# naver-ai/egtr

Hardware: AMD Instinct MI355X
Metric: images/sec end-to-end SGG, 600x1000 input, N=200 queries (higher is better)
Workload: dtype f32; 1 GPU; VG inference: ResNet-50, N=200, 6 enc/6 dec, 150 classes, 50 predicates, 600x1000, bs=1/GPU fp32 (BASELINE configs[1]); hip_graph=True, gemm_tuning=True, miopen_find=True, parallelism=replicas x1 (independent images, no collective)

## Files before the change

### egtr_amd/_lib.py

```python
import ctypes
import os

import torch

_HERE = os.path.dirname(os.path.abspath(__file__))
LIB_PATH = os.environ.get("EGTR_HIP_LIBRARY") or os.path.join(_HERE, "libegtr_hip.so")

_P = ctypes.c_void_p
_I = ctypes.c_int
ABI_VERSION = 5

SIGNATURES = {
    "egtr_abi_version": [],
    "egtr_status_string": [_I],
    "egtr_last_hip_error": [],
    "egtr_msda_forward_f32": [_P, _P, _P, _P, _P, _P, _I, _I, _I, _I, _I, _I, _I, _P],
    "egtr_msda_forward_fused_vbias_f32": [_P, _P, _P, _P, _P, _P, _P, _I, _I, _I, _I, _I, _I, _I, _P, _P, _I, _I, _P, _P,
                                          _P],
    "egtr_msda_forward_fused_box_f32": [_P, _P, _P, _P, _P, _P, _P, _I, _I, _I, _I, _I, _I, _I, _P, _P, _I, _I, _P, _P,
                                        _P],
    "egtr_msda_backward_f32": [_P, _P, _P, _P, _P, _P, _P, _I, _I, _I, _I, _I, _I, _I, _P, _P, _P],
    "egtr_msda_backward_out_f32": [_P, _P, _P, _P, _P, _P, _P, _I, _I, _I, _I, _I, _I, _I, _P, _P, _P],
    "egtr_msda_forward_f64": [_P, _P, _P, _P, _P, _P, _I, _I, _I, _I, _I, _I, _I, _P],
    "egtr_msda_backward_f64": [_P, _P, _P, _P, _P, _P, _P, _I, _I, _I, _I, _I, _I, _I, _P, _P, _P],
# ... 50 lines not shown
                           _I, _P, _P, _P, _P],
    "egtr_oi_match_f32": [_P, _P, _P, _I, _I, _P, _P, _I, _I, _P, _P, ctypes.c_longlong, _P, _P, _P, ctypes.c_longlong,
                          _P, _I, _P, _P, _P],
    "egtr_oi_ap_f64": [_P, _P, _P, _P, ctypes.c_longlong, _I, _P, _P],
    "egtr_coco_match_f32": [_P, _P, _P, _P, _I, _I, _I, _P, _P, _P, _P, _P, ctypes.c_longlong, _P, _P, _I, _P, _P, _P,
                            _P, _P],
    "egtr_coco_accumulate_f64": [_P, _P, _P, _P, _P, ctypes.c_longlong, _I, _P, _P, _P, _P],
    "egtr_hungarian_match_f32": [_P, _P, _P, _P, _P, _P, _P, _I, _I, _I, _I, ctypes.c_float, ctypes.c_float,
                                 ctypes.c_float, _I, ctypes.c_float, ctypes.c_float, _P, _P, _P, _P, _P, _P, _P],
    "egtr_hungarian_match_scratch_doubles": [_I, _I, ctypes.c_longlong],
    "egtr_add_layernorm_backward_f32": [_P, _P, _P, _P, _P, _P, _P, _P, _I, _I, ctypes.c_float],
    "egtr_add_layernorm_backward_workspace_floats": [_I],
    "egtr_msda_geometry_forward_f32": [_P, _P, ctypes.c_longlong, _P, ctypes.c_longlong, _P, _I, _P, _P, _P, ctypes.c_longlong, _I, _I, _I],
    "egtr_msda_geometry_backward_f32": [_P, _P, _P, _P, _P, ctypes.c_longlong, _P, _I, _P, _P, ctypes.c_longlong, _P, ctypes.c_longlong, _P, ctypes.c_longlong, _I, _I, _I],
    "egtr_linear_backward_f32": [_P, _P, _P, _P, _P, ctypes.c_float, _P, _P, _P, _I, _I, _I],
    "egtr_linear_backward_acc_f32": [_P, _P, _P, _P, _P, ctypes.c_float, _P, _P, _P, _I, _I, _I, _P, _P],
    "egtr_weighted_column_sum_f32": [_P, _P, _P, _P, _P, _I, _I],
    "egtr_column_sum_f32": [_P, _P, _P, _P, _P, _P, _I, _I],
    "egtr_column_sum_workspace_floats": [_I, _I],
    "egtr_any_nonfinite_f32": [_P, _P, ctypes.c_longlong, _P],
    "egtr_clamp_if_flag_f32": [_P, _P, _P, ctypes.c_longlong, _P, ctypes.c_float, _I],
    "egtr_detection_loss_f32": [_P, _P, _P, _P, _P, _P, _P, _P, _P, _I, _I, _I, ctypes.c_float, ctypes.c_float, _P, _P,
                                _P, _P],
    "egtr_relation_loss_f32": [_P, _P, _P, _P, _P, _P, _P, _P, _I, _I, _I, ctypes.c_float, _I, _I, _P, _P, _P, _P],
    "egtr_relation_loss_workspace_bytes": [_I, _I],
    "egtr_relation_loss_bits_f32": [_P, _P, _P, _P, _P, _P, _P, _P, _I, _I, _I, ctypes.c_float, _I, _I, _P, _P, _P, _P],
    "egtr_pack_relations_u64": [_P, _P, _P, _I, _I, _I, _I, _P],
    "egtr_rel_head_forward_bf16w": [_P] * 16 + [_I] * 6 + [_P] * 3,
    "egtr_ffn_layernorm_bf16": [_P] * 7 + [ctypes.c_float, _P, _I, _P, _P, _I, _I, _I],
    "egtr_ffn_pack_weights_bf16": [_P, _P, _P, _I, _I, _P],
    "egtr_ffn_packed_weights_bytes": [_I],
    "egtr_linear_bf16": [_P, _P, _I, _P, _P, _P, _I, _I, _I, _I, _I, ctypes.c_float],
    "egtr_rel_head_forward_bf16p": [_P] * 16 + [_I] * 6 + [_P] * 3,
    "egtr_rel_head_pack_tables_bf16": [_P, _P, _I, _I, _I, _P],
    "egtr_linear_split_bf16_f32": [_P, _P, _I, _P, _P, _P, _I, _I, _I, _I, _I],
    "egtr_linear_split_bf16_wgrad_f32": [_P, _P, _I, _P, _I, _P, _P, _I, _I, _I],
    "egtr_linear_split_bf16_wgrad_workspace_floats": [_I, _I, _I],
    "egtr_gemm_split_tile_weights_f32": [_P, _P, _I, _I, _I, _I, _P],
    "egtr_gemm_split_tile_weights_pair_f32": [_P, _P, _I, _I, _I, _P],
    "egtr_gemm_split_tile_weights_multi_f32": [_P, _I, _P, _P, _P, _P, _P, _P, _P, _P],
    "egtr_linear_split_bf16_grouped_pos_f32": [_P, _I, _P, _P, _P, _P, _P, _P, _P, _P, _I, _I, _P, _P],
    "egtr_linear_split_bf16_ex_f32": [_P, _I, _P, _P, _P, _P, _P, _P, _P, _P, _I, _I, _P, _P, _P, _P, _P, _P, _P, _P, _P],
    "egtr_linear_split_bf16_wgrad_ex_f32": [_P, _P, _I, _P, _I, _P, _P, _I, _I, _I, _P, _I, _P],
    "egtr_dropout_add_layernorm_f32": [_P, _P, _P, _P, ctypes.c_float, _P, _P, _P, _I, _I, ctypes.c_float, _P],
    "egtr_dropout_add_layernorm_backward_workspace_floats": [_I],
    "egtr_dropout_add_layernorm_backward_f32": [_P, _P, _P, _P, ctypes.c_float, _P, _P, _P, _P, ctypes.c_float, _P, _P, _P,
                                                _P, _I, _I, ctypes.c_float],
    "egtr_pad_batch_f32": [_P, _P, _P, _I, _I, _I, _I, _P, _P],
    "egtr_preprocess_f32": [_P, _P, _I, _P, _P, _I, _I, _I, _I, _P, _P, _P],
    "egtr_preprocess_bf16": [_P, _P, _I, _P, _P, _I, _I, _I, _I, _P, _P, _P],
    "egtr_preprocess_augment_f32": [_P, _P, _P, _I, _P, _P, _I, _I, _I, _I, _I, _I, _I, _I, _P, _P, _P],
    "egtr_preprocess_augment_bf16": [_P, _P, _P, _I, _P, _P, _I, _I, _I, _I, _I, _I, _I, _I, _P, _P, _P],
    "egtr_conv1x1_tail_x6_f32": [_P, _P, _I, _P, _I, _P, _P, _P, _I, _I, _P, _I, _I, _I, _I, _I, _I],
    "egtr_stem_conv7x7_pool_bf16": [_P, _P, _P, _P, _P, _I, _I, _I],
    "egtr_stem_conv7x7_pool_x6_f32": [_P, _P, _P, _P, _P, _I, _I, _I],
    "egtr_conv1x1_strided_x6_f32": [_P, _P, _P, _P, _I, _I, _I, _I, _I, _I],
    "egtr_conv3x3_phase_channels": [_I, _I, _I, _I],
    "egtr_conv3x3_x6_f32": [_P, _P, _P, _P, _I, _I, _I, _I, _I, _I, _I],
    "egtr_conv3x3_x6_shift_f32": [_P, _P, _P, _P, _P, _I, _I, _I, _I, _I, _I, _I],
    "egtr_conv1x1_tail_pack_weights_bf16": [_P, _P, _I, _I, _I, _P],
    "egtr_conv1x1_tail_bf16": [_P, _P, _I, _P, _I, _P, _P, _P, _I, _I, _P, _I, _I, _I, _I],
    "egtr_ffn_x6_f32": [_P, _P, _I, _P, _P, _P, _P, _P, _P, ctypes.c_float, _P, _I, _P, _P, _I, _I, _I],
    "egtr_encoder_tail_x6_f32": [_P, _P, _I, _P, _I, _P, _P, _P, _P, ctypes.c_float, _P, _P, _P, _P, _P, _P, ctypes.c_float,
                                 _P, _I, _P, _P, _I, _I, _I],
    "egtr_proj_ln_x6_f32": [_P, _P, _I, _P, _P, _P, _I, _P, _P, ctypes.c_float, _P, _I, _P, _P, _I, _I],
    "egtr_proj_multi_x6_f32": [_P, _P, _I, _P, _P, _P, _I, _I, _I],
    "egtr_xs_bytes": [_I, _I],
    "egtr_xs_split_f32": [_P, _P, _I, _P, _I, _I, _I, _P, _P, _I],
    "egtr_rel_head_forward_bf16x6_f32": [_P] * 16 + [_I] * 6 + [_P] * 3 + [_I],
    "egtr_rel_head_forward_bf16x6_save_f32": [_P] * 16 + [_I] * 6 + [_P] * 5,
    "egtr_rel_head_streams_f32": [_P] * 4 + [_I] * 2 + [_P] * 3,
    "egtr_rel_head_forward_save_f32": [_P] * 16 + [_I] * 6 + [_P] * 5,
    "egtr_rel_head_backward_pairs_f32": [_P] * 6 + [_I] * 4 + [_P] * 5,
    "egtr_decoder_layer_f32": [_P, _P],
    "egtr_decoder_layer_workspace": [_I, _I, _P, _P, _P],
}
_RESTYPES = {"egtr_status_string": ctypes.c_char_p, "egtr_last_hip_error": ctypes.c_char_p,
             "egtr_ffn_packed_weights_bytes": ctypes.c_longlong,
             "egtr_input_proj_groupnorm_tokens_workspace_floats": ctypes.c_longlong,
             "egtr_msda_backward_bf16_workspace_floats": ctypes.c_longlong,
             "egtr_hungarian_match_scratch_doubles": ctypes.c_longlong,
             "egtr_relation_loss_workspace_bytes": ctypes.c_longlong,
             "egtr_column_sum_workspace_floats": ctypes.c_longlong,
             "egtr_add_layernorm_backward_workspace_floats": ctypes.c_longlong,
             "egtr_linear_split_bf16_wgrad_workspace_floats": ctypes.c_longlong,
             "egtr_dropout_add_layernorm_backward_workspace_floats": ctypes.c_longlong,
             "egtr_xs_bytes": ctypes.c_longlong, "egtr_sgg_eval_width": ctypes.c_longlong,
             "egtr_oi_eval_width": ctypes.c_longlong, "egtr_matched_topk_workspace_bytes": ctypes.c_longlong, "egtr_oi_select_workspace_bytes": ctypes.c_longlong}

_lib = None


class EgtrHipError(RuntimeError):
    pass


def lib():
    global _lib
    if _lib is None:
        if not os.path.exists(LIB_PATH):
            raise EgtrHipError(
                f"{LIB_PATH} not found: the HIP extension has not been built "
                "(run `make -C egtr_amd/csrc` or __graft_entry__.build()). There is no CPU fallback.")
        handle = ctypes.CDLL(LIB_PATH)
        handle.egtr_abi_version.restype = ctypes.c_int
        got = handle.egtr_abi_version()
# ... 60 lines not shown
```

### egtr_amd/backbone.py

```python
import os

import torch
import torch.nn.functional as F
from torch import nn


TRAIN_FUSED_EPILOGUE = True
NHWC_BF16 = os.environ.get("EGTR_BACKBONE_NHWC", "1") != "0"
NHWC_F32 = os.environ.get("EGTR_BACKBONE_NHWC", "1") != "0"
CONV3_FUSED = True
CONV3_FUSED_BF16 = True
CONV1_X6 = True
CONV1_X6_SHAPES = ((64, 64),)
CONV1_SHIFT_ON_LOAD = True
CONV1_PLAIN_SHAPES = ((256, 64), (256, 128), (512, 128), (1024, 256))
CONV1_SPLIT_SHAPES = ()
SHORTCUT_X6 = True
FROZEN_PREFIX_NHWC = True
STEM_FUSED_BF16 = True
STEM_FUSED = True
CONV2_X6 = True
CONV2_X6_MAX_WIDTH = 512


def _fold(conv, bn):
    scale = bn.weight.float() * (bn.running_var.float() + 1e-5).rsqrt()
    shift = bn.bias.float() - bn.running_mean.float() * scale
    return ((conv.weight.float() * scale.reshape(-1, 1, 1, 1)).to(conv.weight.dtype).contiguous(),
            shift.contiguous())


def conv1x1_as_gemm(x, weight):
    b, c, h, w_ = x.shape
    return torch.matmul(weight.reshape(weight.shape[0], c), x.reshape(b, c, h * w_)).view(b, -1, h, w_)


class DeformableDetrFrozenBatchNorm2d(nn.Module):

    def __init__(self, n):
        super().__init__()
        self.register_buffer("weight", torch.ones(n))
        self.register_buffer("bias", torch.zeros(n))
        self.register_buffer("running_mean", torch.zeros(n))
        self.register_buffer("running_var", torch.ones(n))

    def _load_from_state_dict(self, state_dict, prefix, local_metadata, strict, missing_keys, unexpected_keys,
                              error_msgs):
        state_dict.pop(prefix + "num_batches_tracked", None)
        super()._load_from_state_dict(state_dict, prefix, local_metadata, strict, missing_keys, unexpected_keys,
                                      error_msgs)

    def forward(self, x):
        scale = self.weight * (self.running_var + 1e-5).rsqrt()
        shift = self.bias - self.running_mean * scale
        return x * scale.reshape(1, -1, 1, 1) + shift.reshape(1, -1, 1, 1)


class ScaleWeightsFunction(torch.autograd.Function):

    @staticmethod
    def forward(ctx, scales, *weights):
        from . import ops
        ctx.scales = scales
        return tuple(ops.scale_rows_multi([w.detach() for w in weights], scales))

    @staticmethod
    def backward(ctx, *grads):
        from . import ops
        present = [i for i, g in enumerate(grads) if g is not None]
        out = [None] * len(grads)
# ... 86 lines not shown
        w2, b2 = p[1]
        w3, b3 = p[2]
        out = {"w1": w1.reshape(w1.shape[0], -1).contiguous(), "b1": b1.to(w1.dtype).contiguous(),
               "w2": w2.contiguous(memory_format=torch.channels_last), "b2": b2,
               "w3": w3.reshape(w3.shape[0], -1).contiguous(), "b3": b3, "wd": None}
        if self.downsample is not None:
            wd = p[3][0]
            out["wd"] = (wd.reshape(wd.shape[0], -1).contiguous() if tuple(self.downsample[0].stride) == (1, 1)
                         else wd.contiguous(memory_format=torch.channels_last))
            out["b3"] = p[4][1]
        return out

    def forward_folded_nhwc(self, x, q):
        from . import ops
        B, C, H, W_ = x.shape
        x2 = x.permute(0, 2, 3, 1).reshape(-1, C)
        N1 = q["w1"].shape[0]
        st2 = tuple(self.conv2.stride)
        conv2_x6 = (CONV2_X6 and ops.GEMM_SPLIT_BF16 and st2 in ((1, 1), (2, 2)) and q["w2"].shape[0] <= CONV2_X6_MAX_WIDTH)
        shift1 = None
        if (CONV1_X6 and ops.GEMM_SPLIT_BF16 and (C, N1) in CONV1_X6_SHAPES and ops.conv1x1_tail_supported(x2, N1)):
            if "w1xs" not in q:
                q["w1xs"] = ops.xs_split(q["w1"], weights=True)
                q["b1f"] = q["b1"].float().contiguous()
            y = ops.conv1x1_tail(x2, None, q["w1xs"], q["b1f"], None, N1, relu_in=False, relu_out=True)
        elif (CONV1_SHIFT_ON_LOAD and conv2_x6 and (C, N1) in CONV1_PLAIN_SHAPES and x.is_cuda and x.dtype == torch.float32
              and q["b1"].dtype == torch.float32 and N1 == q["w2"].shape[1]):
            if (C, N1) in CONV1_SPLIT_SHAPES and ops.gemm_split_supported(x2, N1, C):
                if "w1gs" not in q:
                    q["w1gs"] = ops.gemm_split_weights(q["w1"])
                y = ops.linear_split_bf16(x2, q["w1gs"], None, N1)
            else:
                y = torch.mm(x2, q["w1"].t())
            shift1 = q["b1"]
        else:
            y = torch._addmm_activation(q["b1"], x2, q["w1"].t(), use_gelu=False)
        y = y.view(B, H, W_, -1).permute(0, 3, 1, 2)
        conv2_x6 = conv2_x6 and ops.conv3x3_supported(y, q["w2"].shape[0], st2[0])
        if shift1 is not None and not conv2_x6:
            ops.bias_act_rows_(y.permute(0, 2, 3, 1).reshape(-1, N1), shift1)
            shift1 = None
        if conv2_x6:
            if "w2xs" not in q:
                q["w2xs"] = ops.conv3x3_weights(q["w2"], st2[0])
            y = ops.conv3x3(y, q["w2xs"], q["w2"].shape[0], st2[0], in_shift=shift1)
        else:
            y = F.conv2d(y, q["w2"], None, stride=self.conv2.stride, padding=1)
        if not y.is_contiguous(memory_format=torch.channels_last):
            ops.note_fallback("backbone_nhwc", "a channels-last convolution returned an NCHW tensor: "
                              "PYTORCH_MIOPEN_SUGGEST_NHWC=1 was not set before the process's first convolution")
        Ho, Wo = y.shape[-2:]
        y2 = y.permute(0, 2, 3, 1).reshape(-1, y.shape[1])
        N3 = q["w3"].shape[0]
        if self.downsample is None:
            idt = x2
        elif q["wd"].dim() == 2:
            idt = torch.mm(x2, q["wd"].t())
        elif (SHORTCUT_X6 and ops.GEMM_SPLIT_BF16 and tuple(self.downsample[0].stride) == (2, 2)
              and ops.conv1x1_strided_supported(x, N3, 2)):
            if "wdxs" not in q:
                q["wdxs"] = ops.xs_split(q["wd"].reshape(N3, C).contiguous(), weights=True)
            idt = ops.conv1x1_strided(x, q["wdxs"], N3, 2)
        else:
            idt = F.conv2d(x, q["wd"], None, stride=self.downsample[0].stride).permute(0, 2, 3, 1).reshape(-1, N3)
        if (CONV3_FUSED and ops.GEMM_SPLIT_BF16 and ops.conv1x1_tail_supported(y2, N3) and idt.dtype == torch.float32
                and idt.stride(1) == 1 and idt.stride(0) % 4 == 0 and idt.data_ptr() % 16 == 0):
            if "w3xs" not in q:
                q["w3xs"] = ops.xs_split(q["w3"], weights=True)
            z = ops.conv1x1_tail(y2, q["b2"], q["w3xs"], q["b3"], idt, N3)
            return z.view(B, Ho, Wo, -1).permute(0, 3, 1, 2)
        if (CONV3_FUSED_BF16 and ops.conv1x1_tail_bf16_supported(y2, N3) and idt.dtype == torch.bfloat16 and idt.stride(1) == 1
                and idt.stride(0) % 8 == 0 and idt.data_ptr() % 16 == 0):
            if "w3pk" not in q:
                q["w3pk"] = ops.conv_tail_pack_bf16(q["w3"])
            z = ops.conv1x1_tail_bf16(y2, q["b2"], q["w3pk"], q["b3"], idt, N3)
            return z.view(B, Ho, Wo, -1).permute(0, 3, 1, 2)
        ops.bias_act_rows_(y2, q["b2"])
        z = torch.mm(y2, q["w3"].t())
        ops.bias_act_rows_(z, q["b3"], idt)
        return z.view(B, Ho, Wo, -1).permute(0, 3, 1, 2)

    def forward_folded(self, x, p):
        from . import ops
        s = self.conv2.stride
        idt = x
        shift3 = p[2][1]
        if self.downsample is not None:
            if tuple(self.downsample[0].stride) == (1, 1):
                idt = conv1x1_as_gemm(x, p[3][0])
            else:
                idt = F.conv2d(x, p[3][0], None, stride=self.downsample[0].stride)
            shift3 = p[4][1]
        y = ops.bias_act_(conv1x1_as_gemm(x, p[0][0]), p[0][1])
        y = ops.bias_act_(F.conv2d(y, p[1][0], None, stride=s, padding=1), p[1][1])
        return ops.bias_act_(conv1x1_as_gemm(y, p[2][0]), shift3, idt)


class ResNet50Features(nn.Module):

    channels = [512, 1024, 2048]
    reductions = [8, 16, 32]

    def __init__(self, out_indices=(2, 3, 4)):
        super().__init__()
        self.out_indices = tuple(out_indices)
        self.conv1 = nn.Conv2d(3, 64, 7, stride=2, padding=3, bias=False)
# ... 155 lines not shown
```

### egtr_amd/csrc/conv_tail_x6.hip

```cpp
#include <hip/hip_runtime.h>
#include <stdint.h>

#include "common.h"
#include "x6_common.h"
#include "xs_format.h"

namespace {
using namespace x6;
typedef float f32x4v __attribute__((ext_vector_type(4)));

struct TailArgs {
  const float* a;
  const float* a_shift;
  const char* w;
  const float* bias;
  const float* shortcut;
  float* y;
  int M, N, lda, ldsc, ldy;
  int relu_in, relu_out;
  int row_major;
};

__device__ __forceinline__ int xcd_tile(int bid, int total) {
  const int q = total >> 3, r = total & 7, x = bid & 7;
// ... 163 lines not shown
  TAIL_T(t4);
  asm volatile("s_waitcnt vmcnt(0)" ::: "memory");
  TAIL_T(t5);
  if (tid == 0 && blockIdx.x < kTailRecWg) {
    unsigned long long* r = g_tail_rec[blockIdx.x];
    r[0] = rt0;
    r[1] = __builtin_amdgcn_s_memrealtime();
    r[2] = t1 - t0;
    r[3] = t2 - t1;
    r[4] = t3 - t2;
    r[5] = t4 - t3;
    r[6] = t5 - t4;
    r[7] = 1;
  }
#endif
}

template <int BM, int NTW, int KS, int NW = 4>
int launch(hipStream_t st, const TailArgs& A) {
  static unsigned long long raised = 0;
  constexpr int lds = 3 * BM * (16 * KS + 8) * 2;
  auto kern = conv_tail_x6_kernel<BM, NTW, KS, NW>;
  if (lds > 64 * 1024) {
    const int rc = egtr_raise_dynamic_lds(reinterpret_cast<const void*>(kern), lds, &raised);
    if (rc != EGTR_OK) return rc;
  }
  const long long tiles = (long long)((A.M + BM - 1) / BM) * (A.N / (32 * NTW * NW));
  if (tiles >= (1ll << 31)) return EGTR_E_UNSUPPORTED;
  hipLaunchKernelGGL(kern, dim3((unsigned)tiles), dim3(64 * NW), lds, st, A);
  return egtr_check_launch();
}

template <int KS>
int dispatch(hipStream_t st, const TailArgs& A, int force_bm, int force_ntw) {
  if (A.N % 128 != 0) {
    if (force_bm == 64 || force_ntw == 2) return EGTR_E_UNSUPPORTED;
    return launch<32, 1, KS, 2>(st, A);
  }
  const bool n256 = A.N % 256 == 0;
  int bm = 32;
  int ntw = (KS >= 32 && n256) ? 2 : 1;
  if (force_bm) bm = force_bm;
  if (force_ntw) ntw = force_ntw;
  if (ntw == 2 && !n256) return EGTR_E_UNSUPPORTED;
  if (bm == 64 && KS > 16) return EGTR_E_UNSUPPORTED;
  if constexpr (KS <= 16) {
    if (bm == 64) return ntw == 2 ? launch<64, 2, KS>(st, A) : launch<64, 1, KS>(st, A);
  }
  if constexpr (KS >= 32) {
    if (bm == 32 && ntw == 2) return launch<32, 1, KS, 8>(st, A);
  }
  if (bm == 32) return ntw == 2 ? launch<32, 2, KS>(st, A) : launch<32, 1, KS>(st, A);
  return EGTR_E_ARG;
}

}

#ifdef EGTR_TAIL_TIMING
extern "C" int egtr_conv_tail_stamps(unsigned long long* host_out, int reset) {
  if (hipMemcpyFromSymbol(host_out, HIP_SYMBOL(g_tail_rec), sizeof(unsigned long long) * kTailRecWg * 8) != hipSuccess)
    return EGTR_E_LAUNCH;
  if (reset) {
    void* p = nullptr;
    if (hipGetSymbolAddress(&p, HIP_SYMBOL(g_tail_rec)) != hipSuccess ||
        hipMemset(p, 0, sizeof(unsigned long long) * kTailRecWg * 8) != hipSuccess)
      return EGTR_E_LAUNCH;
  }
  return EGTR_OK;
}
#endif

extern "C" int egtr_conv1x1_tail_x6_f32(egtr_stream_t stream, const float* a, int lda, const float* a_shift, int relu_in,
                                        const void* w_xs, const float* bias, const float* shortcut, int ld_shortcut,
                                        int relu_out, float* y, int ldy, int M, int K, int N, int tile_rows, int tile_cols) {
  if (!a || !w_xs || !y || M <= 0 || K <= 0 || N <= 0 || lda < K || ldy < N || (shortcut && ld_shortcut < N)) return EGTR_E_ARG;
  if ((tile_rows != 0 && tile_rows != 32 && tile_rows != 64) || (tile_cols != 0 && tile_cols != 128 && tile_cols != 256))
    return EGTR_E_ARG;
  if ((K != 64 && K != 128 && K != 256 && K != 512) || N % 64 || (lda & 3) || (ldy & 3) || (shortcut && (ld_shortcut & 3)) ||
      (reinterpret_cast<uintptr_t>(a) & 15) || (reinterpret_cast<uintptr_t>(y) & 15) || (reinterpret_cast<uintptr_t>(w_xs) & 15) ||
      (reinterpret_cast<uintptr_t>(a_shift) & 15) || (reinterpret_cast<uintptr_t>(bias) & 15) ||
      (reinterpret_cast<uintptr_t>(shortcut) & 15))
    return EGTR_E_UNSUPPORTED;
  TailArgs A{a, a_shift, static_cast<const char*>(w_xs), bias, shortcut, y, M, N, lda, ld_shortcut, ldy, relu_in, relu_out,
             (long long)M * K * 4 >= (long long)N * K * 6 ? 1 : 0};
  hipStream_t st = static_cast<hipStream_t>(stream);
  const int fn = tile_cols / 128;
  switch (K) {
    case 64: return dispatch<4>(st, A, tile_rows, fn);
    case 128: return dispatch<8>(st, A, tile_rows, fn);
    case 256: return dispatch<16>(st, A, tile_rows, fn);
    default: return dispatch<32>(st, A, tile_rows, fn);
  }
}
```

### egtr_amd/kernels/backbone.py

```python
import torch

from .. import _lib
from .._lib import _chk

__all__ = ["bias_relu_maxpool", "xs_bytes", "xs_split", "conv1x1_tail", "stem_weights", "stem_weights_bf16", "stem_fused_bf16",
           "stem_fused", "conv3x3_weights", "conv3x3", "conv1x1_strided", "conv_tail_pack_bf16", "conv1x1_tail_bf16",
           "bias_act_rows_", "bias_act_"]


def bias_relu_maxpool(x, bias):
    N, C, H, W_ = x.shape
    x2 = _chk(x.contiguous(), "x", torch.float32)
    b2 = _chk(bias.contiguous(), "bias", torch.float32)
    y = torch.empty(N, C, (H - 1) // 2 + 1, (W_ - 1) // 2 + 1, dtype=torch.float32, device=x.device)
    _lib.launch("egtr_bias_relu_maxpool3x3s2_f32", x2.data_ptr(), b2.data_ptr(), y.data_ptr(), N, C, H, W_)
    return y


def xs_bytes(rows, K):
    return int(_lib.lib().egtr_xs_bytes(int(rows), int(K)))


def xs_split(x, pos=None, weights=False, plain=True):
    K = x.shape[-1]
    x2 = _lib.row_view(x, K)
    if not x2.is_cuda or x2.dtype != torch.float32:
        raise RuntimeError("xs_split: x must be a float32 CUDA/HIP tensor")
    rows = x2.shape[0]
    n = xs_bytes(rows, K)
    if n == 0:
        raise RuntimeError(f"xs_split: K = {K} must be a multiple of 16")
    out = torch.empty(n, dtype=torch.uint8, device=x.device) if plain else None
    out_pos, p2 = None, None
    if pos is not None:
        p2 = _chk(pos.reshape(-1, K).contiguous(), "pos", torch.float32)
        out_pos = torch.empty(n, dtype=torch.uint8, device=x.device)
    _lib.launch("egtr_xs_split_f32", x2.data_ptr(), x2.stride(0), _lib.ptr(p2), p2.shape[0] if p2 is not None else 0, rows, K,
                _lib.ptr(out), _lib.ptr(out_pos), 1 if weights else 0)
    return out if pos is None else (out, out_pos)


def conv1x1_tail(a, a_shift, w_xs, bias, shortcut, N, relu_in=True, relu_out=True, tile=(0, 0)):
    M, K = a.shape
    for name, t in (("a_shift", a_shift), ("bias", bias), ("shortcut", shortcut)):
        if t is not None and (not t.is_cuda or t.dtype != torch.float32 or t.stride(-1) != 1):
            raise RuntimeError(f"conv1x1_tail: {name} must be a float32 device tensor with unit inner stride")
    y = torch.empty(M, N, dtype=torch.float32, device=a.device)
    _lib.launch("egtr_conv1x1_tail_x6_f32", a.data_ptr(), a.stride(0), _lib.ptr(a_shift), 1 if relu_in else 0, w_xs.data_ptr(),
                _lib.ptr(bias), _lib.ptr(shortcut), shortcut.stride(0) if shortcut is not None else 0, 1 if relu_out else 0,
                y.data_ptr(), y.stride(0), M, K, N, int(tile[0]), int(tile[1]))
    return y


def stem_weights(w):
    wm = torch.zeros(64, 7, 8, 4, dtype=torch.float32, device=w.device)
    wm[:, :, :7, :3] = w.detach().permute(0, 2, 3, 1)
    return xs_split(wm.reshape(64, 224), weights=True)


def stem_weights_bf16(w):
    wm = torch.zeros(64, 7, 8, 4, dtype=torch.bfloat16, device=w.device)
    wm[:, :, :7, :3] = w.detach().permute(0, 2, 3, 1)
    return conv_tail_pack_bf16(wm.reshape(64, 224).contiguous())


def stem_fused_bf16(x, w_packed, bias):
    B, _, H, W = x.shape
    Hc, Wc = (H - 1) // 2 + 1, (W - 1) // 2 + 1
    Hp, Wp = (Hc - 1) // 2 + 1, (Wc - 1) // 2 + 1
    y = torch.empty((B, 64, Hp, Wp), dtype=torch.bfloat16, device=x.device, memory_format=torch.channels_last)
    _lib.launch("egtr_stem_conv7x7_pool_bf16", x.data_ptr(), w_packed.data_ptr(), bias.data_ptr(), y.data_ptr(), B, H, W)
    return y


def stem_fused(x, w_xs, bias):
    B, _, H, W = x.shape
    Hc, Wc = (H - 1) // 2 + 1, (W - 1) // 2 + 1
    Hp, Wp = (Hc - 1) // 2 + 1, (Wc - 1) // 2 + 1
    y = torch.empty((B, 64, Hp, Wp), dtype=torch.float32, device=x.device, memory_format=torch.channels_last)
    _lib.launch("egtr_stem_conv7x7_pool_x6_f32", x.data_ptr(), w_xs.data_ptr(), bias.data_ptr(), y.data_ptr(), B, H, W)
    return y


def conv3x3_weights(w, stride=1, variant=0):
    N, C = w.shape[:2]
    cp = int(_lib.lib().egtr_conv3x3_phase_channels(int(C), int(N), int(stride), int(variant)))
    if cp <= 0:
        raise RuntimeError(f"conv3x3_weights: C = {C}, N = {N}, stride {stride} is not served")
    wm = w.detach().reshape(N, C // cp, cp, 3, 3).permute(0, 1, 3, 4, 2).reshape(N, 9 * C).contiguous()
    return xs_split(wm, weights=True)


def conv3x3(x, w_xs, N, stride=1, variant=0, in_shift=None):
    B, C, H, W = x.shape
    Ho, Wo = (H - 1) // stride + 1, (W - 1) // stride + 1
    y = torch.empty((B, N, Ho, Wo), dtype=torch.float32, device=x.device, memory_format=torch.channels_last)
    if in_shift is None:
        _lib.launch("egtr_conv3x3_x6_f32", x.data_ptr(), w_xs.data_ptr(), y.data_ptr(), B, H, W, C, N, int(stride), int(variant))
        return y
    if (not in_shift.is_cuda or in_shift.dtype != torch.float32 or in_shift.dim() != 1 or in_shift.shape[0] != C
            or not in_shift.is_contiguous()):
        raise RuntimeError(f"conv3x3: in_shift must be a contiguous float32 [{C}] device tensor")
    _lib.launch("egtr_conv3x3_x6_shift_f32", x.data_ptr(), in_shift.data_ptr(), w_xs.data_ptr(), y.data_ptr(), B, H, W, C, N,
# ... 68 lines not shown
```

### egtr_amd/ops.py

```python
import os

import torch
from torch.autograd import Function
from torch.autograd.function import once_differentiable

from . import _lib
from . import targets as rel_targets
from ._lib import _chk, _stream
from .kernels.backbone import *
from .kernels.derived import *
from .kernels.elementwise import *
from .kernels.elementwise import _DIM_T
from .kernels.heads import *
from .kernels.linear import *
from .kernels.linear import _c16, _host_array, _skinny_bwd, _skinny_fwd, _split3_bf16, _wgrad_ex
from .kernels.protocols import *
from .kernels.statistics import *
from .kernels.vrd import *
from .load_custom import load_hip_kernels

_MSDA = None


def _msda():
# ... 696 lines not shown
ENV_ROUTE_SWITCHES = ("EGTR_DECODER_CLUSTER", "EGTR_GEMM_SPLIT_BF16", "EGTR_REL_HEAD_SPLIT_BF16", "EGTR_FFN_FUSED",
                      "EGTR_BACKBONE_NHWC", "EGTR_ENCODER_TRAIN_FUSED", "EGTR_TOKEN_LINEAR")

FALLBACKS = {}
STRICT_FAST_PATH = os.environ.get("EGTR_STRICT_FAST_PATH", "0") == "1"


class FastPathError(RuntimeError):
    pass


def note_fallback(name, why=""):
    n = FALLBACKS.get(name, 0)
    FALLBACKS[name] = n + 1
    if STRICT_FAST_PATH:
        raise FastPathError(f"left the HIP fast path '{name}': {why}")
    if n == 0:
        import warnings
        warnings.warn(f"egtr_amd: leaving the HIP fast path '{name}' ({why}); counted in egtr_amd.ops.FALLBACKS",
                      RuntimeWarning, stacklevel=3)


def _gate(name, eligible, ok, why):
    if eligible and not ok:
        note_fallback(name, why() if callable(why) else why)
    return bool(ok)


def inference_fast_path(x):
    return x.is_cuda and x.dtype == torch.float32 and not torch.is_grad_enabled()


DEFER_LAYERNORM = True

GEMM_SPLIT_BF16 = os.environ.get("EGTR_GEMM_SPLIT_BF16", "1") != "0"
LAZY_POS = True
GEMM_SPLIT_MIN_ROWS = 4096
GEMM_SPLIT_WGRAD = True


def gemm_split_supported(x, N, K):
    rows = x.numel() // x.shape[-1]
    eligible = (GEMM_SPLIT_BF16 and x.is_cuda and x.dtype == torch.float32 and not torch.is_grad_enabled()
                and rows >= GEMM_SPLIT_MIN_ROWS)
    return _gate("gemm_split", eligible, eligible and K % 32 == 0 and N % 128 == 0,
                 lambda: f"{rows} x {K} -> {N}: K must be a multiple of 32 and N of 128 (vendor GEMM instead)")


def conv1x1_tail_supported(a, N):
    return (a.is_cuda and a.dtype == torch.float32 and a.dim() == 2 and a.stride(1) == 1 and a.stride(0) % 4 == 0
            and a.data_ptr() % 16 == 0 and a.shape[1] in (64, 128, 256, 512) and N % 64 == 0)


def stem_fused_bf16_supported(x, w):
    return (x.is_cuda and x.dtype == torch.bfloat16 and x.dim() == 4 and x.shape[1] == 3 and x.is_contiguous()
            and tuple(w.shape) == (64, 3, 7, 7) and w.dtype == torch.bfloat16)


def stem_fused_supported(x, w):
    return (x.is_cuda and x.dtype == torch.float32 and x.dim() == 4 and x.shape[1] == 3 and x.is_contiguous()
            and tuple(w.shape) == (64, 3, 7, 7))


def conv3x3_supported(x, N, stride=1, variant=0):
    return (x.is_cuda and x.dtype == torch.float32 and x.dim() == 4 and x.is_contiguous(memory_format=torch.channels_last)
            and x.data_ptr() % 16 == 0
            and int(_lib.lib().egtr_conv3x3_phase_channels(int(x.shape[1]), int(N), int(stride), int(variant))) > 0)


def conv1x1_strided_supported(x, N, stride):
    return (x.is_cuda and x.dtype == torch.float32 and x.dim() == 4 and x.is_contiguous(memory_format=torch.channels_last)
            and x.data_ptr() % 16 == 0 and x.shape[1] in (256, 512, 1024) and N % 128 == 0 and stride in (1, 2))


def conv1x1_tail_bf16_supported(a, N):
    return (a.is_cuda and a.dtype == torch.bfloat16 and a.dim() == 2 and a.stride(1) == 1 and a.stride(0) % 8 == 0
            and a.data_ptr() % 16 == 0 and a.shape[1] in (64, 128, 256, 512) and N % 256 == 0)


FFN_FUSED = os.environ.get("EGTR_FFN_FUSED", "1") != "0"


def ffn_fused_supported(x, fc1, fc2, ln):
    rows = x.numel() // x.shape[-1]
    eligible = FFN_FUSED and GEMM_SPLIT_BF16 and inference_fast_path(x) and rows >= GEMM_SPLIT_MIN_ROWS
    ok = (eligible and x.shape[-1] == 256 and tuple(fc1.weight.shape)[1] == 256 and fc1.weight.shape[0] % 64 == 0
          and tuple(fc2.weight.shape) == (256, fc1.weight.shape[0]) and fc1.bias is not None and fc2.bias is not None
          and ln.weight.shape[0] == 256 and fc1.weight.dtype == torch.float32)
    return _gate("ffn_fused", eligible, ok,
                 lambda: f"d_model {x.shape[-1]}, fc1 {tuple(fc1.weight.shape)}: the row-panel kernel serves d_model 256, "
                         "a hidden width that is a multiple of 64, biases present")


ENCODER_TAIL_FUSED = True


def encoder_tail_fused_supported(context, out_proj, ln1, fc1, fc2, ln2):
    return (ENCODER_TAIL_FUSED and proj_ln_fused_supported(context, out_proj, ln1)
            and ffn_fused_supported(context, fc1, fc2, ln2))


def proj_ln_fused_supported(x, lin, ln):
    rows = x.numel() // x.shape[-1]
    eligible = FFN_FUSED and GEMM_SPLIT_BF16 and inference_fast_path(x) and rows >= GEMM_SPLIT_MIN_ROWS
    ok = (eligible and x.shape[-1] == 256 and tuple(lin.weight.shape) == (256, 256) and lin.bias is not None
          and ln.weight.shape[0] == 256 and lin.weight.dtype == torch.float32)
# ... 432 lines not shown
```

### include/egtr_hip.h

```cpp
#ifndef EGTR_HIP_H
#define EGTR_HIP_H

#include <stdint.h>

#ifdef __cplusplus
extern "C" {
#endif

typedef void* egtr_stream_t;

enum {
  EGTR_OK = 0,
  EGTR_E_ARG = -1,
  EGTR_E_LAUNCH = -2,
  EGTR_E_UNSUPPORTED = -3
};

#define EGTR_ABI_VERSION 5
int egtr_abi_version(void);
const char* egtr_status_string(int status);
const char* egtr_last_hip_error(void);

int egtr_msda_forward_f32(egtr_stream_t stream, const float* value, const int64_t* spatial_shapes,
                          const int64_t* level_start_index, const float* sampling_loc, const float* attn_weight,
// ... 336 lines not shown
                                float* gate_mean);

int egtr_rel_head_pack_tables_bf16(egtr_stream_t stream, const void* u ,
                                   int u_is_bf16, int rows, int num_slots, uint16_t* packed);
int egtr_rel_head_forward_bf16p(egtr_stream_t stream, const float* gate_q, const float* gate_k,
                                const uint16_t* uq_packed, const uint16_t* uk_packed, const float* b1,
                                const uint16_t* w2r, const float* b2r, const uint16_t* w3r, const float* b3r,
                                const uint16_t* w2c, const float* b2c, const uint16_t* w3c, const float* b3c,
                                const float* triplet_dist, const int64_t* node_cls, int batch, int num_query,
                                int num_slots, int hidden, int num_rel, int num_cls_plus1, float* rel_logits,
                                float* conn_logits, float* gate_mean);

int egtr_linear_bf16(egtr_stream_t stream, const uint16_t* x, int ldx, const uint16_t* weight, const uint16_t* bias,
                     uint16_t* y, int ldy, int M, int N, int K, int relu, float alpha);

int egtr_linear_split_bf16_f32(egtr_stream_t stream, const float* x, int ldx, const uint16_t* w_tiled,
                               const float* bias, float* y, int ldy, int M, int K, int N, int relu);

int egtr_gemm_split_tile_weights_f32(egtr_stream_t stream, const float* w, int ldw, int transposed, int N, int K,
                                     uint16_t* w_tiled);
int egtr_gemm_split_tile_weights_pair_f32(egtr_stream_t stream, const float* w, int ldw, int N, int K,
                                          uint16_t* w_tiled_pair);
int egtr_gemm_split_tile_weights_multi_f32(egtr_stream_t stream, int num_weights, const float* const* w, const int* ldw,
                                           const float* const* w2, const int* ldw2, const int* split_rows, const int* N,
                                           const int* K, uint16_t* const* w_tiled_pair);

long long egtr_linear_split_bf16_wgrad_workspace_floats(int M, int N, int K);
int egtr_linear_split_bf16_wgrad_f32(egtr_stream_t stream, const float* g, int ldg, const float* x, int ldx,
                                     float* grad_weight, float* workspace, int M, int N, int K);

int egtr_linear_split_bf16_grouped_pos_f32(egtr_stream_t stream, int num_problems, const float* const* x, const int* ldx,
                                           const uint16_t* const* w_tiled, const float* const* bias, float* const* y,
                                           const int* ldy, const int* N, const int* relu, int M, int K,
                                           const float* const* pos, const int* pos_rows);

int egtr_linear_split_bf16_ex_f32(egtr_stream_t stream, int num_problems, const float* const* x, const int* ldx,
                                  const uint16_t* const* w_tiled, const float* const* bias, float* const* y,
                                  const int* ldy, const int* N, const int* relu, int M, int K, const float* const* pos,
                                  const int* pos_rows, const unsigned char* const* row_keep, const float* const* relu_ref,
                                  const int* ldref, const float* const* add1, const float* const* add2, const int* ldadd,
                                  float* const* colpart);
int egtr_linear_split_bf16_wgrad_ex_f32(egtr_stream_t stream, const float* g, int ldg, const float* x, int ldx,
                                        float* grad_weight, float* workspace, int M, int N, int K, const float* x_pos,
                                        int pos_rows, const unsigned char* row_keep);

long long egtr_xs_bytes(int rows, int K);
int egtr_xs_split_f32(egtr_stream_t stream, const float* x, int ldx, const float* pos, int pos_rows, int rows, int K,
                      void* xs_out, void* xs_pos_out, int round_to_nearest);

int egtr_conv1x1_tail_x6_f32(egtr_stream_t stream, const float* a, int lda, const float* a_shift, int relu_in,
                             const void* w_xs, const float* bias, const float* shortcut, int ld_shortcut, int relu_out,
                             float* y, int ldy, int M, int K, int N, int tile_rows, int tile_cols);

int egtr_stem_conv7x7_pool_x6_f32(egtr_stream_t stream, const float* x, const void* w_xs, const float* bias, float* y, int B,
                                  int H, int W);

int egtr_stem_conv7x7_pool_bf16(egtr_stream_t stream, const uint16_t* x, const uint16_t* w_packed, const float* bias, uint16_t* y,
                                int B, int H, int W);

int egtr_conv3x3_phase_channels(int C, int N, int stride, int variant);
int egtr_conv3x3_x6_f32(egtr_stream_t stream, const float* x, const void* w_xs, float* y, int B, int H, int W, int C, int N,
                        int stride, int variant);
int egtr_conv3x3_x6_shift_f32(egtr_stream_t stream, const float* x, const float* in_shift, const void* w_xs, float* y, int B, int H,
                              int W, int C, int N, int stride, int variant);

int egtr_conv1x1_strided_x6_f32(egtr_stream_t stream, const float* x, const void* w_xs, float* y, int B, int H, int W, int C, int N,
                                int stride);

int egtr_conv1x1_tail_pack_weights_bf16(egtr_stream_t stream, const uint16_t* w, int ldw, int N, int K, uint16_t* w_packed);
int egtr_conv1x1_tail_bf16(egtr_stream_t stream, const uint16_t* a, int lda, const float* a_shift, int relu_in,
                           const uint16_t* w_packed, const float* bias, const uint16_t* shortcut, int ld_shortcut, int relu_out,
                           uint16_t* y, int ldy, int M, int K, int N);

int egtr_ffn_x6_f32(egtr_stream_t stream, const float* x, int ldx, const void* w1_xs, const float* b1, const void* w2_xs,
                    const float* b2, const float* ln_gamma, const float* ln_beta, float eps, const float* pos,
                    int pos_rows, float* out, float* out_pos, int M, int d_model, int ffn_dim);

long long egtr_ffn_packed_weights_bytes(int ffn_dim);
int egtr_ffn_pack_weights_bf16(egtr_stream_t stream, const uint16_t* w1, const uint16_t* w2, int d_model, int ffn_dim,
                               uint16_t* packed);
int egtr_ffn_layernorm_bf16(egtr_stream_t stream, const uint16_t* x, const uint16_t* w_packed, const uint16_t* b1,
                            const uint16_t* b2, const uint16_t* gamma, const uint16_t* beta, float eps, const uint16_t* pos,
                            int pos_rows, uint16_t* y, uint16_t* y_pos, int M, int d_model, int ffn_dim);

int egtr_encoder_tail_x6_f32(egtr_stream_t stream, const float* context, int ldc, const float* hidden, int ldh,
                             const void* wp_xs, const float* bp, const float* ln1_gamma, const float* ln1_beta, float eps1,
                             const void* w1_xs, const float* b1, const void* w2_xs, const float* b2, const float* ln2_gamma,
                             const float* ln2_beta, float eps2, const float* pos, int pos_rows, float* out, float* out_pos,
                             int M, int d_model, int ffn_dim);

int egtr_proj_ln_x6_f32(egtr_stream_t stream, const float* x, int ldx, const void* w_xs, const float* bias,
                        const float* residual, int ldr, const float* ln_gamma, const float* ln_beta, float eps,
                        const float* pos, int pos_rows, float* out, float* out_pos, int M, int d_model);

int egtr_proj_multi_x6_f32(egtr_stream_t stream, const float* x, int ldx, const void* w_xs, const float* bias, float* out,
                           int M, int d_model, int num_weights);

int egtr_rel_head_forward_bf16x6_f32(egtr_stream_t stream, const float* gate_q, const float* gate_k, const float* uq,
                                     const float* uk, const float* b1, const uint16_t* w2x_rel, const float* b2r,
                                     const uint16_t* w3x_rel, const float* b3r, const uint16_t* w2x_conn,
                                     const float* b2c, const float* w3c, const float* b3c, const float* triplet_dist,
                                     const int64_t* node_cls, int batch, int num_query, int num_slots, int hidden,
                                     int num_rel, int num_cls_plus1, float* rel_logits, float* conn_logits,
                                     float* gate_mean, int apply_sigmoid);

int egtr_rel_head_forward_bf16x6_save_f32(egtr_stream_t stream, const float* gate_q, const float* gate_k, const float* uq,
// ... 62 lines not shown
```

Baseline: 401.7 images/sec.

## Fold projection shortcut GEMM into the conv1x1 tail kernel via concatenated K

Result: no change. 405.3 images/sec (median of 6 runs) (+0.9%).

```diff
diff --git a/egtr_amd/_lib.py b/egtr_amd/_lib.py
--- a/egtr_amd/_lib.py
+++ b/egtr_amd/_lib.py
@@ -126,6 +126,7 @@
     "egtr_preprocess_augment_f32": [_P, _P, _P, _I, _P, _P, _I, _I, _I, _I, _I, _I, _I, _I, _P, _P, _P],
     "egtr_preprocess_augment_bf16": [_P, _P, _P, _I, _P, _P, _I, _I, _I, _I, _I, _I, _I, _I, _P, _P, _P],
     "egtr_conv1x1_tail_x6_f32": [_P, _P, _I, _P, _I, _P, _P, _P, _I, _I, _P, _I, _I, _I, _I, _I, _I],
+    "egtr_conv1x1_tail_sc_x6_f32": [_P, _P, _I, _P, _I, _P, _I, _I, _I, _I, _I, _P, _P, _I, _P, _I, _I, _I, _I, _I],
     "egtr_stem_conv7x7_pool_bf16": [_P, _P, _P, _P, _P, _I, _I, _I],
     "egtr_stem_conv7x7_pool_x6_f32": [_P, _P, _P, _P, _P, _I, _I, _I],
     "egtr_conv1x1_strided_x6_f32": [_P, _P, _P, _P, _I, _I, _I, _I, _I, _I],
diff --git a/egtr_amd/backbone.py b/egtr_amd/backbone.py
--- a/egtr_amd/backbone.py
+++ b/egtr_amd/backbone.py
@@ -16,6 +16,8 @@
 CONV1_PLAIN_SHAPES = ((256, 64), (256, 128), (512, 128), (1024, 256))
 CONV1_SPLIT_SHAPES = ()
 SHORTCUT_X6 = True
+SHORTCUT_IN_TAIL = True
+SHORTCUT_IN_TAIL_SHAPES = ((64, 64),)
 FROZEN_PREFIX_NHWC = True
 STEM_FUSED_BF16 = True
 STEM_FUSED = True
@@ -208,6 +210,13 @@
         Ho, Wo = y.shape[-2:]
         y2 = y.permute(0, 2, 3, 1).reshape(-1, y.shape[1])
         N3 = q["w3"].shape[0]
+        if (self.downsample is not None and SHORTCUT_IN_TAIL and CONV3_FUSED and SHORTCUT_X6 and ops.GEMM_SPLIT_BF16
+                and (C, y2.shape[1]) in SHORTCUT_IN_TAIL_SHAPES and q["w3"].dtype == torch.float32
+                and ops.conv1x1_tail_sc_supported(y2, x, N3, self.downsample[0].stride[0])):
+            if "w3dxs" not in q:
+                q["w3dxs"] = ops.xs_split(torch.cat([q["w3"], q["wd"].reshape(N3, C)], 1).contiguous(), weights=True)
+            z = ops.conv1x1_tail(y2, q["b2"], q["w3dxs"], q["b3"], None, N3, proj=(x, self.downsample[0].stride[0]))
+            return z.view(B, Ho, Wo, -1).permute(0, 3, 1, 2)
         if self.downsample is None:
             idt = x2
         elif q["wd"].dim() == 2:
diff --git a/egtr_amd/csrc/conv_tail_x6.hip b/egtr_amd/csrc/conv_tail_x6.hip
--- a/egtr_amd/csrc/conv_tail_x6.hip
+++ b/egtr_amd/csrc/conv_tail_x6.hip
@@ -239,6 +239,196 @@
   }
   if (bm == 32) return ntw == 2 ? launch<32, 2, KS>(st, A) : launch<32, 1, KS>(st, A);
   return EGTR_E_ARG;
+}
+
+
+struct TailScArgs {
+  const float* a;
+  const float* a_shift;
+  const float* x;
+  const char* w;
+  const float* bias;
+  float* y;
+  int M, N, lda, ldy;
+  int H, W, Ho, Wo, stride;
+  int relu_in, relu_out;
+  int row_major;
+};
+
+template <int NTW, int KS1, int KS2, int NW, int KP>
+__global__ __launch_bounds__(64 * NW) void conv_tail_sc_x6_kernel(TailScArgs A) {
+  constexpr int BM = 32;
+  constexpr int K1 = 16 * KS1, K2 = 16 * KS2, KS = KS1 + KS2;
+  constexpr int BN = 32 * NTW * NW;
+  constexpr int NT = 64 * NW;
+  constexpr int kPitch = KP + 8;
+  constexpr int C4 = KP / 4;
+  constexpr int RS = NT / C4;
+  constexpr int NQ = BM * C4 / NT;
+  constexpr int KSP = KP / 16;
+  constexpr int NP1 = K1 / KP, NP = (K1 + K2) / KP;
+  constexpr int PF = EGTR_TAIL_PF_LONG;
+  static_assert(K1 % KP == 0 && K2 % KP == 0, "a phase reads one source");
+  static_assert(NT % C4 == 0 && NQ >= 1 && NQ <= 8, "a thread keeps one column group, and one phase of it in registers");
+  static_assert(KSP % 2 == 0 && KSP > PF, "operand double buffer; the weight queue is shorter than a phase");
+  extern __shared__ __attribute__((aligned(16))) char s_raw[];
+  __bf16* const sA = reinterpret_cast<__bf16*>(s_raw);
+
+  const int tid = threadIdx.x, lane = tid & 63, li = lane & 31, hf = lane >> 5;
+  const int wave = __builtin_amdgcn_readfirstlane(tid >> 6);
+  const int mblocks = (A.M + BM - 1) / BM;
+  const int tile = xcd_tile(blockIdx.x, gridDim.x);
+  const int nblocks = A.N / BN;
+  const int nb = A.row_major ? tile % nblocks : tile / mblocks;
+  const int m0 = (A.row_major ? tile / nblocks : tile - nb * mblocks) * BM;
+  const int nt0 = nb * (BN / 32) + wave * NTW;
+
+  const int c4 = tid % C4, r0 = tid / C4;
+  int pix[NQ];
+#pragma unroll
+  for (int q = 0; q < NQ; ++q) {
+    const int row = min(m0 + r0 + RS * q, A.M - 1);
+    if (A.stride == 1) {
+      pix[q] = row;
+    } else {
+      const unsigned t = (unsigned)row / (unsigned)A.Wo, wo = (unsigned)row - t * A.Wo;
+      const unsigned b = t / (unsigned)A.Ho, ho = t - b * A.Ho;
+      pix[q] = (int)((b * A.H + ho * A.stride) * A.W + wo * A.stride);
+    }
+  }
+  f32x4v v[NQ];
+  f32x4v sh = {0.f, 0.f, 0.f, 0.f};
+  auto request_panel = [&](auto p_) {
+    constexpr int p = decltype(p_)::value;
+    if constexpr (p < NP1) {
+#pragma unroll
+      for (int q = 0; q < NQ; ++q) {
+        const int row = min(m0 + r0 + RS * q, A.M - 1);
+        v[q] = *reinterpret_cast<const f32x4v*>(A.a + (size_t)row * A.lda + p * KP + 4 * c4);
+      }
+      if (A.a_shift != nullptr) sh = *reinterpret_cast<const f32x4v*>(A.a_shift + p * KP + 4 * c4);
+    } else {
+#pragma unroll
+      for (int q = 0; q < NQ; ++q)
+        v[q] = *reinterpret_cast<const f32x4v*>(A.x + (size_t)pix[q] * K2 + (p - NP1) * KP + 4 * c4);
+    }
+  };
+  const bool relu_in = A.relu_in != 0;
+  auto park_panel = [&](auto p_) {
+    constexpr int p = decltype(p_)::value;
+#pragma unroll
+    for (int q = 0; q < NQ; ++q) {
+      f32x4v t = v[q];
+      if constexpr (p < NP1) {
+        t = t + sh;
+        if (relu_in) t = f32x4v{egtr_relu(t.x), egtr_relu(t.y), egtr_relu(t.z), egtr_relu(t.w)};
+      }
+      const xs::Split3 s0 = xs::split3_fast(t.x), s1 = xs::split3_fast(t.y), s2 = xs::split3_fast(t.z),
+                       s3 = xs::split3_fast(t.w);
+      __bf16* p0 = sA + (r0 + RS * q) * kPitch + 4 * c4;
+      *reinterpret_cast<uint2*>(p0) = make_uint2(xs::pack_hi16(s0.hi, s1.hi), xs::pack_hi16(s2.hi, s3.hi));
+      *reinterpret_cast<uint2*>(p0 + BM * kPitch) = make_uint2(xs::pack_hi16(s0.mid, s1.mid), xs::pack_hi16(s2.mid, s3.mid));
+      *reinterpret_cast<uint2*>(p0 + 2 * BM * kPitch) = make_uint2(xs::pack_hi16(s0.lo, s1.lo), xs::pack_hi16(s2.lo, s3.lo));
+    }
+  };
+
+  request_panel(std::integral_constant<int, 0>{});
+  __builtin_amdgcn_sched_barrier(0);
+  const char* const wlane = A.w + (size_t)nt0 * KS * (3 * xs::kFragBytes) + lane * 16;
+  bf16x8 w[PF + 1][NTW][3];
+  auto load_w = [&](int ks, bf16x8 (&dst)[NTW][3]) {
+#pragma unroll
+    for (int t = 0; t < NTW; ++t)
+#pragma unroll
+      for (int p = 0; p < 3; ++p)
+        dst[t][p] = *reinterpret_cast<const bf16x8*>(wlane + ((size_t)(t * KS + ks) * 3 + p) * xs::kFragBytes);
+  };
+  static_for<PF>([&](auto i_) {
+    constexpr int i = decltype(i_)::value;
+    load_w(i, w[i]);
+  });
+  float bz[NTW];
+#pragma unroll
+  for (int t = 0; t < NTW; ++t) bz[t] = A.bias != nullptr ? A.bias[(nt0 + t) * 32 + li] : 0.f;
+  __builtin_amdgcn_sched_barrier(0);
+
+  f32x16 acc[NTW];
+#pragma unroll
+  for (int t = 0; t < NTW; ++t)
+#pragma unroll
+    for (int r = 0; r < 16; ++r) acc[t][r] = 0.f;
+
+  const __bf16* const pa0 = sA + li * kPitch + 8 * hf;
+  bf16x8 a[2][3];
+  auto read_a = [&](int j, bf16x8 (&dst)[3]) {
+#pragma unroll
+    for (int p = 0; p < 3; ++p) dst[p] = *reinterpret_cast<const bf16x8*>(pa0 + p * BM * kPitch + 16 * j);
+  };
+  static_for<NP>([&](auto p_) {
+    constexpr int p = decltype(p_)::value;
+    park_panel(p_);
+    __syncthreads();
+    if constexpr (p + 1 < NP) request_panel(std::integral_constant<int, p + 1>{});
+    read_a(0, a[0]);
+    static_for<KSP>([&](auto j_) {
+      constexpr int j = decltype(j_)::value, ks = p * KSP + j;
+      if constexpr (ks + PF < KS) load_w(ks + PF, w[(ks + PF) % (PF + 1)]);
+      if constexpr (j + 1 < KSP) read_a(j + 1, a[(j + 1) & 1]);
+      __builtin_amdgcn_sched_barrier(0);
+#pragma unroll
+      for (int t = 0; t < NTW; ++t) acc[t] = mfma6(a[j & 1], w[ks % (PF + 1)][t], acc[t]);
+      __builtin_amdgcn_sched_barrier(0);
+    });
+    if constexpr (p + 1 < NP) __syncthreads();
+  });
+
+  const bool relu_out = A.relu_out != 0;
+#pragma unroll
+  for (int t = 0; t < NTW; ++t) {
+    const int col = (nt0 + t) * 32 + li;
+    const float b = bz[t];
+#pragma unroll
+    for (int r = 0; r < 16; ++r) {
+      const int row = m0 + (r & 3) + 8 * (r >> 2) + 4 * hf;
+      float o = acc[t][r] + b;
+      if (relu_out) o = egtr_relu(o);
+      if (row < A.M) A.y[(size_t)row * A.ldy + col] = o;
+    }
+  }
+}
+
+template <int NTW, int KS1, int KS2, int NW, int KP>
+int launch_sc(hipStream_t st, const TailScArgs& A) {
+  static unsigned long long raised = 0;
+  constexpr int lds = 3 * 32 * (KP + 8) * 2;
+  auto kern = conv_tail_sc_x6_kernel<NTW, KS1, KS2, NW, KP>;
+  if (lds > 64 * 1024) {
+    const int rc = egtr_raise_dynamic_lds(reinterpret_cast<const void*>(kern), lds, &raised);
+    if (rc != EGTR_OK) return rc;
+  }
+  const long long tiles = (long long)((A.M + 31) / 32) * (A.N / (32 * NTW * NW));
+  if (tiles >= (1ll << 31)) return EGTR_E_UNSUPPORTED;
+  hipLaunchKernelGGL(kern, dim3((unsigned)tiles), dim3(64 * NW), lds, st, A);
+  return egtr_check_launch();
+}
+
+template <int KS1, int KS2>
+int dispatch_sc(hipStream_t st, const TailScArgs& A, int force_bm, int force_ntw) {
+  constexpr int K1 = 16 * KS1;
+  if (force_bm == 64) return EGTR_E_UNSUPPORTED;
+  if (A.N % 128 != 0) {
+    if (force_ntw == 2) return EGTR_E_UNSUPPORTED;
+    return launch_sc<1, KS1, KS2, 2, (K1 < 128 ? K1 : 128)>(st, A);
+  }
+  const bool n256 = A.N % 256 == 0;
+  int ntw = (KS1 >= 32 && n256) ? 2 : 1;
+  if (force_ntw) ntw = force_ntw;
+  if (ntw == 2 && !n256) return EGTR_E_UNSUPPORTED;
+  if constexpr (KS1 >= 32) {
+    if (ntw == 2) return launch_sc<1, KS1, KS2, 8, K1>(st, A);
+  }
+  constexpr int KP = K1 < 256 ? K1 : 256;
+  return ntw == 2 ? launch_sc<2, KS1, KS2, 4, KP>(st, A) : launch_sc<1, KS1, KS2, 4, KP>(st, A);
 }
 
 }
@@ -279,3 +469,29 @@
     default: return dispatch<32>(st, A, tile_rows, fn);
   }
 }
+
+extern "C" int egtr_conv1x1_tail_sc_x6_f32(egtr_stream_t stream, const float* a, int lda, const float* a_shift, int relu_in,
+                                           const float* x, int B, int H, int W, int K2, int stride, const void* w_xs,
+                                           const float* bias, int relu_out, float* y, int ldy, int K1, int N, int tile_rows,
+                                           int tile_cols) {
+  if (!a || !x || !w_xs || !y || B <= 0 || H <= 0 || W <= 0 || K1 <= 0 || K2 <= 0 || N <= 0 || lda < K1 || ldy < N)
+    return EGTR_E_ARG;
+  if ((tile_rows != 0 && tile_rows != 32 && tile_rows != 64) || (tile_cols != 0 && tile_cols != 128 && tile_cols != 256))
+    return EGTR_E_ARG;
+  if ((stride != 1 && stride != 2) || N % 64 || (lda & 3) || (ldy & 3) || (reinterpret_cast<uintptr_t>(a) & 15) ||
+      (reinterpret_cast<uintptr_t>(x) & 15) || (reinterpret_cast<uintptr_t>(y) & 15) || (reinterpret_cast<uintptr_t>(w_xs) & 15) ||
+      (reinterpret_cast<uintptr_t>(a_shift) & 15) || (reinterpret_cast<uintptr_t>(bias) & 15) ||
+      (long long)B * H * W >= (1ll << 31))
+    return EGTR_E_UNSUPPORTED;
+  const int Ho = (H - 1) / stride + 1, Wo = (W - 1) / stride + 1;
+  const int M = B * Ho * Wo;
+  TailScArgs A{a, a_shift, x, static_cast<const char*>(w_xs), bias, y, M, N, lda, ldy, H, W, Ho, Wo, stride, relu_in, relu_out,
+               (long long)M * 4 >= (long long)N * 6 ? 1 : 0};
+  hipStream_t st = static_cast<hipStream_t>(stream);
+  const int fn = tile_cols / 128;
+  if (K1 == 64 && K2 == 64) return dispatch_sc<4, 4>(st, A, tile_rows, fn);
+  if (K1 == 128 && K2 == 256) return dispatch_sc<8, 16>(st, A, tile_rows, fn);
+  if (K1 == 256 && K2 == 512) return dispatch_sc<16, 32>(st, A, tile_rows, fn);
+  if (K1 == 512 && K2 == 1024) return dispatch_sc<32, 64>(st, A, tile_rows, fn);
+  return EGTR_E_UNSUPPORTED;
+}
diff --git a/egtr_amd/kernels/backbone.py b/egtr_amd/kernels/backbone.py
--- a/egtr_amd/kernels/backbone.py
+++ b/egtr_amd/kernels/backbone.py
@@ -3,7 +3,7 @@
 from .. import _lib
 from .._lib import _chk
 
-__all__ = ["bias_relu_maxpool", "xs_bytes", "xs_split", "conv1x1_tail", "stem_weights", "stem_weights_bf16", "stem_fused_bf16",
+__all__ = ["bias_relu_maxpool", "xs_bytes", "xs_split", "conv1x1_tail", "conv1x1_tail_sc", "stem_weights", "stem_weights_bf16", "stem_fused_bf16",
            "stem_fused", "conv3x3_weights", "conv3x3", "conv1x1_strided", "conv_tail_pack_bf16", "conv1x1_tail_bf16",
            "bias_act_rows_", "bias_act_"]
 
@@ -40,7 +40,11 @@
     return out if pos is None else (out, out_pos)
 
 
-def conv1x1_tail(a, a_shift, w_xs, bias, shortcut, N, relu_in=True, relu_out=True, tile=(0, 0)):
+def conv1x1_tail(a, a_shift, w_xs, bias, shortcut, N, relu_in=True, relu_out=True, tile=(0, 0), proj=None):
+    if proj is not None:
+        if shortcut is not None:
+            raise RuntimeError("conv1x1_tail: the shortcut is given either as values or as the projection to fold in, not both")
+        return conv1x1_tail_sc(a, a_shift, w_xs, bias, proj[0], proj[1], N, relu_in=relu_in, relu_out=relu_out, tile=tile)
     M, K = a.shape
     for name, t in (("a_shift", a_shift), ("bias", bias), ("shortcut", shortcut)):
         if t is not None and (not t.is_cuda or t.dtype != torch.float32 or t.stride(-1) != 1):
@@ -49,6 +53,23 @@
     _lib.launch("egtr_conv1x1_tail_x6_f32", a.data_ptr(), a.stride(0), _lib.ptr(a_shift), 1 if relu_in else 0, w_xs.data_ptr(),
                 _lib.ptr(bias), _lib.ptr(shortcut), shortcut.stride(0) if shortcut is not None else 0, 1 if relu_out else 0,
                 y.data_ptr(), y.stride(0), M, K, N, int(tile[0]), int(tile[1]))
+    return y
+
+
+def conv1x1_tail_sc(a, a_shift, w_xs, bias, x, stride, N, relu_in=True, relu_out=True, tile=(0, 0)):
+    M, K1 = a.shape
+    if (not x.is_cuda or x.dtype != torch.float32 or x.dim() != 4 or not x.is_contiguous(memory_format=torch.channels_last)):
+        raise RuntimeError("conv1x1_tail_sc: x must be a dense channels-last float32 [B, C, H, W] device tensor")
+    B, K2, H, W = x.shape
+    if B * ((H - 1) // stride + 1) * ((W - 1) // stride + 1) != M:
+        raise RuntimeError(f"conv1x1_tail_sc: a has {M} rows, x {tuple(x.shape)} at stride {stride} has another number of pixels")
+    for name, t in (("a", a), ("a_shift", a_shift), ("bias", bias)):
+        if t is not None and (not t.is_cuda or t.dtype != torch.float32 or t.stride(-1) != 1):
+            raise RuntimeError(f"conv1x1_tail_sc: {name} must be a float32 device tensor with unit inner stride")
+    y = torch.empty(M, N, dtype=torch.float32, device=a.device)
+    _lib.launch("egtr_conv1x1_tail_sc_x6_f32", a.data_ptr(), a.stride(0), _lib.ptr(a_shift), 1 if relu_in else 0, x.data_ptr(),
+                B, H, W, K2, int(stride), w_xs.data_ptr(), _lib.ptr(bias), 1 if relu_out else 0, y.data_ptr(), y.stride(0), K1, N,
+                int(tile[0]), int(tile[1]))
     return y
 
 
diff --git a/egtr_amd/ops.py b/egtr_amd/ops.py
--- a/egtr_amd/ops.py
+++ b/egtr_amd/ops.py
@@ -772,6 +772,18 @@
             and a.data_ptr() % 16 == 0 and a.shape[1] in (64, 128, 256, 512) and N % 64 == 0)
 
 
+TAIL_SC_KK = ((64, 64), (128, 256), (256, 512), (512, 1024))
+
+
+def conv1x1_tail_sc_supported(a, x, N, stride):
+    if not (conv1x1_tail_supported(a, N) and x.is_cuda and x.dtype == torch.float32 and x.dim() == 4
+            and x.is_contiguous(memory_format=torch.channels_last) and x.data_ptr() % 16 == 0 and stride in (1, 2)
+            and (a.shape[1], x.shape[1]) in TAIL_SC_KK):
+        return False
+    B, _, H, W = x.shape
+    return B * ((H - 1) // stride + 1) * ((W - 1) // stride + 1) == a.shape[0] and B * H * W < 2 ** 31
+
+
 def stem_fused_bf16_supported(x, w):
     return (x.is_cuda and x.dtype == torch.bfloat16 and x.dim() == 4 and x.shape[1] == 3 and x.is_contiguous()
             and tuple(w.shape) == (64, 3, 7, 7) and w.dtype == torch.bfloat16)
diff --git a/include/egtr_hip.h b/include/egtr_hip.h
--- a/include/egtr_hip.h
+++ b/include/egtr_hip.h
@@ -412,6 +412,10 @@
                              const void* w_xs, const float* bias, const float* shortcut, int ld_shortcut, int relu_out,
                              float* y, int ldy, int M, int K, int N, int tile_rows, int tile_cols);
 
+int egtr_conv1x1_tail_sc_x6_f32(egtr_stream_t stream, const float* a, int lda, const float* a_shift, int relu_in, const float* x,
+                                int B, int H, int W, int K2, int stride, const void* w_xs, const float* bias, int relu_out,
+                                float* y, int ldy, int K1, int N, int tile_rows, int tile_cols);
+
 int egtr_stem_conv7x7_pool_x6_f32(egtr_stream_t stream, const float* x, const void* w_xs, const float* bias, float* y, int B,
                                   int H, int W);
 
```
